# wyf0912/ContextGS

Hardware: AMD Instinct MI355X
Metric: views/sec fwd+bwd @1920×1080, 1M anchors (higher is better)
Workload: dtype f32

## Files before the change

contextgs_amd/_lib.py:

```python
from __future__ import annotations

import ctypes as C
import os
import threading

_HERE = os.path.dirname(os.path.abspath(__file__))
LIB_PATH = os.environ.get("CGS_LIB_PATH") or os.path.join(_HERE, "libcgs_hip.so")

_lib = None
_lock = threading.Lock()

c_void_p, c_int, c_int32, c_int64, c_size_t, c_float = C.c_void_p, C.c_int, C.c_int32, C.c_int64, C.c_size_t, C.c_float


class RasterCfg(C.Structure):
    _fields_ = [
        ("image_height", c_int32),
        ("image_width", c_int32),
        ("tanfovx", c_float),
        ("tanfovy", c_float),
        ("scale_modifier", c_float),
        ("prefiltered", c_int32),
        ("debug", c_int32),
        ("viewmatrix", c_void_p),
# ... 16 lines not shown
        ("step_size", c_float),
        ("bias2_sqrt", c_float),
        ("eps", c_float),
        ("weight_decay", c_float),
    ]


class RateSubLevel(C.Structure):
    _fields_ = [("in_dim", c_int32), ("use_clamp", c_int32), ("n", c_int64), ("m", c_int64)] + [
        (k, c_void_p) for k in ("X", "loc", "W1", "b1", "W2", "b2", "yf", "ys", "yo", "Q", "masks", "x_means", "sums3", "g_sums3",
                                "side_f", "side_s", "side_o", "side_Q", "dx_sub", "d_masks", "dW1", "db1", "dW2", "db2")]


_BWD_HEAD = [C.POINTER(RasterCfg), c_int64, c_int64]
_BWD_WS = [c_void_p, c_size_t, c_void_p, c_size_t, c_void_p, c_size_t]
_BWD_TAIL = [c_void_p, c_size_t, c_void_p]
_BWD_FORMS = _BWD_HEAD + [c_void_p] * 3 + [c_int32] * 2 + [c_void_p] * 5 + _BWD_WS + [c_void_p]
_BWD_MAPS = _BWD_FORMS + [c_void_p] * 3
_BWD_OUT = [c_void_p] * 8 + _BWD_TAIL
_BWD_FEAT = [c_void_p, c_int32, c_void_p, c_void_p]

SIGNATURES = {
    "cgs_version": (c_int, []),
    "cgs_last_error": (C.c_char_p, []),
    "cgs_filter": (c_int, [C.POINTER(RasterCfg), c_int64, c_void_p, c_void_p, c_void_p, c_void_p, c_void_p]),
    "cgs_filter_voxel": (c_int, [C.POINTER(RasterCfg), c_int64, c_void_p, c_void_p, c_int64, c_int, c_void_p, c_void_p, c_void_p]),
    "cgs_raster_geom_bytes": (c_size_t, [c_int64]),
    "cgs_raster_bin_bytes": (c_size_t, [c_int64, c_int64]),
    "cgs_raster_img_bytes": (c_size_t, [c_int32, c_int32]),
    "cgs_raster_bwd_scratch_bytes": (c_size_t, [c_int64]),
    "cgs_raster_preprocess": (c_int, [C.POINTER(RasterCfg), c_int64, c_void_p, c_void_p, c_void_p, c_void_p,
                                      c_void_p, c_void_p, c_size_t, c_void_p, C.POINTER(c_int64), c_void_p]),
    "cgs_raster_preprocess_launch": (c_int, [C.POINTER(RasterCfg), c_int64, c_void_p, c_void_p, c_void_p, c_void_p,
                                             c_void_p, c_void_p, c_size_t, c_void_p, c_void_p, C.POINTER(C.c_uint64)]),
    "cgs_raster_preprocess_launch_ex": (c_int, [C.POINTER(RasterCfg), c_int64, c_void_p, c_void_p, c_void_p, c_int32, c_int32,
                                                c_void_p, c_void_p, c_void_p, c_void_p, c_void_p, c_size_t, c_void_p, c_void_p,
                                                C.POINTER(C.c_uint64)]),
    "cgs_raster_backward_ex": (c_int, _BWD_FORMS + _BWD_OUT),
    "cgs_raster_render_aux": (c_int, [C.POINTER(RasterCfg), c_int64, c_int64, c_void_p, c_size_t, c_void_p, c_size_t,
                                      c_void_p, c_size_t, c_void_p, c_void_p, c_void_p, c_void_p]),
    "cgs_raster_backward_aux": (c_int, _BWD_MAPS + _BWD_OUT),
    "cgs_raster_bwd_aux_scratch_bytes": (c_size_t, [c_int64]),
    "cgs_raster_preprocess_launch_opt": (c_int, [C.POINTER(RasterCfg), c_int64, c_void_p, c_void_p, c_void_p, c_int32, c_int32,
                                                 c_void_p, c_void_p, c_void_p, c_void_p, c_void_p, c_size_t, c_void_p, c_void_p,
                                                 C.POINTER(C.c_uint64), C.c_uint32]),
    "cgs_raster_backward_opt": (c_int, _BWD_MAPS + _BWD_OUT + [C.c_uint32]),
    "cgs_raster_render_features": (c_int, [C.POINTER(RasterCfg), c_int64, c_int64, c_void_p, c_size_t, c_void_p, c_size_t,
                                           c_void_p, c_size_t, c_void_p, c_int32, c_void_p, c_void_p]),
    "cgs_raster_backward_feat": (c_int, _BWD_MAPS + _BWD_OUT + [C.c_uint32] + _BWD_FEAT),
    "cgs_raster_bwd_abs_scratch_bytes": (c_size_t, [c_int64]),
    "cgs_raster_backward_abs": (c_int, _BWD_MAPS + _BWD_OUT + [C.c_uint32] + _BWD_FEAT),
    "cgs_raster_bwd_det_bytes": (c_size_t, [c_int64, c_int64, c_int32]),
    "cgs_raster_backward_det": (c_int, _BWD_MAPS + _BWD_OUT + [C.c_uint32, c_int32, c_void_p, c_size_t]),
    "cgs_raster_render_geom": (c_int, [C.POINTER(RasterCfg), c_int64, c_int64, c_void_p, c_size_t, c_void_p, c_size_t,
                                       c_void_p, c_size_t, c_void_p, c_void_p, c_void_p, c_void_p, c_void_p]),
    "cgs_raster_backward_geom": (c_int, _BWD_MAPS + _BWD_OUT + [C.c_uint32] + _BWD_FEAT + [c_void_p] * 4),
    "cgs_raster_contrib": (c_int, [C.POINTER(RasterCfg), c_int64, c_int64, c_void_p, c_size_t, c_void_p, c_size_t, c_void_p,
                                   c_size_t, c_void_p, c_int64] + [c_void_p] * 8),
    "cgs_raster_camera_bytes": (c_size_t, [c_int64]),
    "cgs_raster_camera_backward": (c_int, [C.POINTER(RasterCfg), c_int64, c_void_p, c_void_p, c_int32, c_int32, c_void_p, c_void_p,
                                           c_void_p, c_void_p, c_void_p, c_void_p, c_size_t, c_void_p, c_void_p, C.c_uint32,
                                           c_void_p, c_void_p, c_void_p, c_void_p, c_size_t, c_void_p]),
    "cgs_gaussian_normals_fwd": (c_int, [C.POINTER(RasterCfg), c_int64] + [c_void_p] * 5),
    "cgs_gaussian_normals_bwd": (c_int, [C.POINTER(RasterCfg), c_int64] + [c_void_p] * 6),
    "cgs_depth_normals_fwd": (c_int, [c_int32, c_int32, c_float, c_float, c_float] + [c_void_p] * 3),
    "cgs_depth_normals_bwd": (c_int, [c_int32, c_int32, c_float, c_float, c_float] + [c_void_p] * 4),
    "cgs_normal_consistency_fwd": (c_int, [c_int32, c_int32, c_float, c_float, c_float] + [c_void_p] * 5),
    "cgs_normal_consistency_bwd": (c_int, [c_int32, c_int32, c_float, c_float, c_float] + [c_void_p] * 7),
    "cgs_filter_cov": (c_int,[C.POINTER(RasterCfg), c_int64, c_void_p, c_void_p, c_void_p, c_void_p]),
    "cgs_raster_preprocess_wait": (c_int, [C.c_uint64, C.POINTER(c_int64)]),
    "cgs_raster_preprocess_wait2": (c_int, [C.c_uint64, C.POINTER(c_int64), C.POINTER(c_int)]),
    "cgs_debug_set_depth_keys_full": (c_int, [c_int]),
    "cgs_sort_depth_keys": (c_int, [c_void_p, c_void_p, c_void_p, c_void_p, c_void_p, c_int64, c_void_p, c_size_t, c_void_p,
                                    C.c_uint32, c_void_p]),
    "cgs_raster_render_spec": (c_int, [C.POINTER(RasterCfg), c_int64, c_int64, c_void_p, c_size_t, c_void_p, c_size_t,
                                       c_void_p, c_size_t, c_void_p, c_void_p]),
    "cgs_raster_render": (c_int, [C.POINTER(RasterCfg), c_int64, c_int64, c_void_p, c_size_t, c_void_p, c_size_t,
                                  c_void_p, c_size_t, c_void_p, c_void_p]),
    "cgs_raster_backward": (c_int, _BWD_HEAD + [c_void_p] * 6 + _BWD_WS + [c_void_p] * 7 + _BWD_TAIL),
    "cgs_raster_preprocess_expand_launch": (c_int, [C.POINTER(RasterCfg), c_int64, c_int] + [c_void_p] * 9 + [c_int64, c_void_p,
                                                    c_void_p, c_void_p, c_void_p, c_size_t, c_void_p, c_void_p, C.POINTER(C.c_uint64)]),
    "cgs_raster_stats": (c_int, [C.POINTER(RasterCfg), c_void_p, c_size_t, c_void_p, c_void_p]),
    "cgs_debug_set_bin_mode": (c_int, [c_int]),
    "cgs_debug_bin_compare": (c_int, [C.POINTER(RasterCfg), c_int64, c_int64, c_int64, c_void_p, c_size_t, c_void_p, c_size_t,
                                      c_void_p, c_size_t, c_void_p, c_size_t, c_void_p, c_void_p, c_void_p]),
    "cgs_build_info": (C.c_char_p, []),
    "cgs_scan_scratch_bytes": (c_size_t, [c_int64]),
    "cgs_scan_exclusive_u32": (c_int, [c_void_p, c_void_p, c_int64, c_void_p, c_size_t, c_void_p]),
    "cgs_sort_scratch_bytes": (c_size_t, [c_int64]),
    "cgs_sort_pairs_u32": (c_int, [c_void_p, c_void_p, c_void_p, c_void_p, c_void_p, c_void_p, c_int64, c_int, c_int,
                                   c_void_p, c_size_t, c_void_p]),
    "cgs_quantize_anchor": (c_int, [c_void_p, c_void_p, c_void_p, c_int64, c_int, c_void_p, c_void_p, c_void_p]),
    "cgs_ste_multistep": (c_int, [c_void_p, c_void_p, c_int64, c_int64, c_int, c_void_p, c_void_p]),
    "cgs_entropy_gaussian_fwd": (c_int, [c_void_p, c_void_p, c_void_p, c_void_p, c_int64, c_int64, c_void_p, c_int,
                                         c_void_p, c_void_p]),
    "cgs_entropy_gaussian_bwd": (c_int, [c_void_p, c_void_p, c_void_p, c_void_p, c_int64, c_int64, c_void_p, c_int,
                                         c_void_p, c_void_p, c_void_p, c_void_p, c_void_p, c_void_p]),
    "cgs_mlp2_forward": (c_int, [c_int, c_int, c_int, c_int, c_void_p, c_int64, c_void_p, c_void_p, c_void_p, c_void_p,
                                 c_void_p, c_int64, c_void_p, c_int64, c_void_p]),
    "cgs_mlp2_backward": (c_int, [c_int, c_int, c_int, c_int, c_void_p, c_int64, c_void_p, c_void_p, c_void_p, c_void_p, c_void_p,
                                  c_int64, c_void_p, c_void_p, c_int64, c_int, c_void_p, c_void_p, c_void_p, c_void_p,
                                  c_void_p, c_void_p, c_int64, c_void_p, c_size_t, c_void_p]),
    "cgs_mlp2_backward_rows": (c_int, [c_int, c_int, c_int, c_int, c_void_p, c_int64, c_void_p, c_void_p, c_void_p, c_void_p,
                                       c_void_p, c_int64, c_void_p, c_void_p, c_int64, c_int, c_void_p, c_void_p, c_void_p,
                                       c_void_p, c_void_p, c_void_p, c_void_p, c_int64, c_void_p, c_size_t, c_void_p]),
    "cgs_mlp_wgrad_scratch_bytes": (c_size_t, []),
    "cgs_mlp2_wgrad": (c_int, [c_int, c_int, c_int, c_void_p, c_int64, c_void_p, c_void_p, c_int64, c_void_p, c_void_p, c_void_p,
                               c_void_p, c_void_p, c_int64, c_void_p, c_size_t, c_void_p]),
    "cgs_anchor_mlp3_wgrad": (c_int, [c_void_p, c_int64] + [c_void_p] * 9 + [c_int64, c_void_p, c_size_t, c_void_p]),
    "cgs_anchor_mlp3_forward": (c_int, [c_void_p, c_int64, c_void_p, c_void_p, c_void_p, c_void_p, c_void_p, c_void_p,
                                        c_void_p, c_void_p, c_int64, c_void_p]),
    "cgs_anchor_mlp3_backward": (c_int, [c_void_p, c_int64, c_void_p, c_void_p, c_void_p, c_void_p, c_void_p, c_void_p,
                                         c_void_p, c_void_p, c_void_p, c_int64, c_void_p, c_void_p, c_void_p, c_void_p,
                                         c_void_p, c_void_p, c_void_p, c_int64, c_void_p, c_size_t, c_void_p]),
    "cgs_anchor_mlp3_forward_rows": (c_int, [c_void_p] * 13 + [c_int64, c_void_p]),
    "cgs_anchor_mlp3_backward_rows": (c_int, [c_void_p] * 22 + [c_int64, c_void_p, c_size_t, c_void_p]),
    "cgs_anchor_mlp3_forward_rows_t": (c_int, [c_void_p] * 13 + [c_int64, c_int, c_void_p]),
    "cgs_anchor_mlp3_backward_rows_t": (c_int, [c_void_p] * 22 + [c_int64, c_int, c_void_p, c_size_t, c_void_p]),
    "cgs_rowcat_fwd": (c_int, [c_int, c_void_p, c_void_p, c_void_p, c_void_p, c_int64, c_void_p, c_void_p]),
    "cgs_rowcat_bwd": (c_int, [c_int, c_void_p, c_void_p, c_void_p, c_void_p, c_void_p, c_int64, c_void_p, c_void_p]),
    "cgs_anchor_mlp3_layout": (c_int, [c_void_p]),
    "cgs_gather_rows_segmented": (c_int, [c_int, c_void_p, c_void_p, c_void_p, c_void_p, c_int64, c_int, c_void_p, c_void_p]),
    "cgs_scatter_rows_sorted": (c_int, [c_void_p, c_void_p, c_int64, c_int64, c_int, c_void_p, c_void_p]),
    "cgs_add_rows": (c_int, [c_void_p, c_void_p, c_int64, c_int64, c_int, c_void_p, c_void_p]),
    "cgs_weighted_sum_scratch_bytes": (c_size_t, []),
    "cgs_weighted_sum_fwd": (c_int, [c_void_p, c_void_p, c_int64, c_void_p, c_float, c_void_p, c_size_t, c_void_p, c_void_p]),
    "cgs_weighted_sum_bwd": (c_int, [c_void_p, c_void_p, c_int64, c_float, c_void_p, c_void_p, c_void_p]),
    "cgs_gather_rows": (c_int, [c_void_p, c_void_p, c_int64, c_int, c_void_p, c_void_p]),
    "cgs_mark_rows": (c_int, [c_void_p, c_int64, c_int64, C.c_uint32, c_void_p, c_void_p]),
    "cgs_zero_unmarked_rows": (c_int, [c_void_p, C.c_uint32, c_int64, c_int, c_void_p, c_void_p, c_void_p]),
    "cgs_rowcat_fwd_masked": (c_int, [c_int, c_void_p, c_void_p, c_void_p, c_void_p, c_void_p, c_int64, c_void_p, c_void_p]),
    "cgs_rowcat_bwd_masked": (c_int, [c_int, c_void_p, c_void_p, c_void_p, c_void_p, c_void_p, c_void_p, c_int64, c_void_p,
                                      c_void_p]),
    "cgs_ctx_gather_bwd": (c_int, [c_void_p, c_int64, c_int64, c_void_p, c_void_p, c_void_p, c_void_p, c_void_p, c_void_p,
                                   c_int, c_int, c_int, c_void_p]),
    "cgs_ctx_gather_bwd_acc": (c_int, [c_void_p, c_int64, c_int64, c_void_p, c_void_p, c_void_p, c_void_p, c_void_p, c_void_p,
                                       c_int, c_int, c_int, c_int, c_void_p]),
    "cgs_noise_quant_fwd": (c_int, [c_void_p, c_void_p, c_void_p, c_void_p, c_void_p, c_int64, c_int, c_int, c_int,
                                    C.c_uint64, c_float, c_float, c_float, c_void_p, c_void_p, c_void_p, c_void_p,
                                    c_void_p, c_void_p]),
    "cgs_hyper_noise_gather": (c_int, [c_void_p, c_void_p, c_int64, c_int, C.c_uint64, c_void_p, c_void_p]),
    "cgs_eb_bits_scratch_bytes": (c_size_t, []),
    "cgs_eb_bits_fwd": (c_int, [c_void_p, c_void_p, c_void_p, c_int64, c_int, c_void_p, c_size_t, c_void_p, c_void_p]),
    "cgs_eb_bits_bwd": (c_int, [c_void_p, c_void_p, c_void_p, c_void_p, c_int64, c_int, c_void_p, c_void_p, c_void_p]),
    "cgs_rate_finish_fwd": (c_int, [c_void_p, c_int, c_void_p, c_float, C.c_double, C.c_double, C.c_double, c_float, c_void_p,
                                    c_void_p, c_void_p]),
    "cgs_rate_finish_bwd": (c_int, [c_void_p, c_int, c_float, C.c_double, C.c_double, C.c_double, c_void_p, c_void_p, c_void_p]),
    "cgs_rate_finish_bwd4": (c_int, [c_void_p, c_void_p, c_void_p, c_void_p, c_int, c_float, C.c_double, C.c_double, C.c_double, c_void_p,
                                     c_void_p, c_void_p]),
    "cgs_ctx_choose_blocks": (c_size_t, [c_int64]),
    "cgs_ctx_choose_flags": (c_int, [c_void_p, c_int64, c_void_p, c_void_p, C.c_uint64, c_float, c_void_p, c_void_p, c_void_p,
                                     c_void_p, c_int, c_void_p, c_void_p, c_void_p, c_void_p]),
    "cgs_ctx_choose_slot_ints": (c_int, []),
    "cgs_ctx_choose_flags_slots": (c_int, [c_void_p, c_int64, c_void_p, c_void_p, C.c_uint64, c_float, c_void_p, c_void_p, c_void_p,
                                           c_void_p, c_int, c_void_p, c_void_p, c_void_p, c_int, c_void_p]),
    "cgs_ctx_choose_compact": (c_int, [c_void_p, c_void_p, c_void_p, c_int64, c_void_p, c_int, c_void_p, c_void_p, c_void_p,
                                       c_void_p, c_void_p, c_void_p]),
    "cgs_means_accum_doubles": (c_size_t, []),
    "cgs_means_finalize": (c_int, [c_void_p, c_int64, c_int64, c_int64, c_void_p, c_void_p]),
    "cgs_noise_quant_bwd": (c_int, [c_void_p, c_void_p, c_void_p, c_void_p, c_void_p, c_int64, c_int, c_int, c_int,
                                    C.c_uint64, c_float, c_float, c_float, c_void_p, c_void_p, c_void_p, c_void_p,
                                    c_void_p, c_void_p, c_void_p, c_void_p, c_void_p, c_void_p, c_void_p]),
    "cgs_ctx_level_fwd": (c_int, [c_int, c_void_p, c_int64, c_void_p, c_void_p, c_void_p, c_void_p, c_int64, c_void_p, c_void_p,
                                  c_int64] + [c_void_p] * 8 + [C.c_uint64, c_float, c_float, c_float] + [c_void_p] * 7),
    "cgs_ctx_level_bwd_scratch_bytes": (c_size_t, []),
    "cgs_ctx_level_bwd": (c_int, [c_int] + [c_void_p] * 9 + [c_int64, C.c_uint64, c_float, c_float, c_float, c_void_p, c_int64] +
# ... 183 lines not shown
```

contextgs_amd/csrc/tile_bin.hip:

```cpp
#include "cgs_internal.h"
#include "buf_access.h"

#define TB_THREADS 256
#define TB_ITEMS 16
#define TB_TILE (TB_THREADS * TB_ITEMS)
#define TB_WAVES (TB_THREADS / CGS_WAVE)
#define TB_MAXR 256
#ifndef TB_XCD_MAP
#define TB_XCD_MAP 0
#endif

int cgs_scan_exclusive_u32_total(const uint32_t *in, uint32_t *out, int64_t n, void *scratch, size_t scratch_bytes,
                                 uint32_t *grand_total, hipStream_t stream);

namespace {

#ifndef GR_ITEMS
#define GR_ITEMS 2
#endif
__global__ void __launch_bounds__(256)
    gather_rects_kernel(int64_t P, const uint32_t *__restrict__ order, const uint2 *__restrict__ rect,
                        uint32_t *__restrict__ rect_lo, uint32_t *__restrict__ rect_hi, uint32_t *__restrict__ cnt) {
    const int64_t blk = cgs_xcd_item((P + 256 * GR_ITEMS - 1) / (256 * GR_ITEMS));
    if (blk < 0) return;
// ... 9 lines not shown
        const int64_t i = i0 + 256 * k;
        if (i < P) {
            rect_lo[i] = rc[k].x;
            rect_hi[i] = rc[k].y;
            const uint32_t w = (rc[k].y & 0xFFFFu) - (rc[k].x & 0xFFFFu), h = (rc[k].y >> 16) - (rc[k].x >> 16);
            cnt[i] = w * h;
        }
    }
}

__global__ void __launch_bounds__(256)
    block_first_kernel(int64_t nb, int64_t P, const uint32_t *__restrict__ offsets, uint32_t *__restrict__ bf, int nt,
                       uint2 *__restrict__ ranges, const uint32_t *__restrict__ R_dev, uint32_t R_cap) {
    const int64_t b = (int64_t)blockIdx.x * 256 + threadIdx.x;
    if (b < nt) ranges[b] = make_uint2(0u, 0u);
    if (R_dev) nb = ((int64_t)min(*R_dev, R_cap) + TB_TILE - 1) / TB_TILE;
    if (b > nb) return;
    if (b == nb) { bf[b] = (uint32_t)(P - 1); return; }
    const uint32_t target = (uint32_t)(b * TB_TILE);
    int64_t lo = 0, hi = P;
    while (lo < hi) {
        const int64_t mid = (lo + hi) >> 1;
        if (offsets[mid] <= target) lo = mid + 1; else hi = mid;
    }
    bf[b] = (uint32_t)(lo - 1);
}

__device__ __forceinline__ void build_owner_index(uint32_t *sidx, uint32_t *swave , uint32_t base, uint32_t i_lo,
                                                  uint32_t i_hi, int64_t P, uint32_t R,
                                                  const uint32_t *__restrict__ offsets) {
    const int tid = threadIdx.x, lane = tid & 63, wave = tid >> 6;
#pragma unroll
    for (int k = 0; k < TB_ITEMS; ++k) sidx[k * TB_THREADS + tid] = 0u;
    __syncthreads();
    for (uint32_t i = i_lo + 1u + (uint32_t)tid; i <= i_hi; i += TB_THREADS) {
        const uint32_t o = offsets[i];
        const uint32_t on = (int64_t)i + 1 < P ? offsets[i + 1] : R;
        if (on > o && o > base && o - base < (uint32_t)TB_TILE) sidx[o - base] = i - i_lo;
    }
    __syncthreads();
    uint32_t v[TB_ITEMS];
    uint32_t run = 0;
#pragma unroll
    for (int k = 0; k < TB_ITEMS; ++k) {
        v[k] = sidx[tid * TB_ITEMS + k];
        run = max(run, v[k]);
    }
    uint32_t inc = run;
#pragma unroll
    for (int d = 1; d < 64; d <<= 1) {
        const uint32_t o = (uint32_t)__shfl_up((int)inc, d, 64);
        if (lane >= d) inc = max(inc, o);
    }
    if (lane == 63) swave[wave] = inc;
    __syncthreads();
    uint32_t pre = (uint32_t)__shfl_up((int)inc, 1, 64);
    if (lane == 0) pre = 0;
#pragma unroll
    for (int w = 0; w < TB_WAVES; ++w) pre = (w < wave) ? max(pre, swave[w]) : pre;
    run = pre;
#pragma unroll
    for (int k = 0; k < TB_ITEMS; ++k) {
        run = max(run, v[k]);
        sidx[tid * TB_ITEMS + k] = run;
    }
    __syncthreads();
}

struct TbPair { uint32_t key, i, mask; };

#define BK_W 8
#define BK_H 4
#define BK_TILES (BK_W * BK_H)

__device__ __forceinline__ void bucket_rect(uint32_t lo, uint32_t hi, uint32_t &cx0, uint32_t &cy0, uint32_t &cw, uint32_t &ch) {
    const uint32_t x0 = lo & 0xFFFFu, y0 = lo >> 16, x1 = hi & 0xFFFFu, y1 = hi >> 16;
    const bool some = x1 > x0 && y1 > y0;
    cx0 = x0 / BK_W;
    cy0 = y0 / BK_H;
    cw = some ? (x1 + BK_W - 1) / BK_W - cx0 : 0u;
    ch = some ? (y1 + BK_H - 1) / BK_H - cy0 : 0u;
}

template <bool COARSE>
__device__ __forceinline__ TbPair gen_pair(uint32_t j, uint32_t base, uint32_t i_lo, const uint32_t *sidx,
                                           const uint32_t *__restrict__ offsets, const uint32_t *__restrict__ rect_lo,
                                           const uint32_t *__restrict__ rect_hi, uint32_t tiles_x) {
    TbPair p;
    p.i = i_lo + sidx[j - base];
    p.mask = 0u;
    const uint32_t local = j - offsets[p.i];
    const uint32_t lo = rect_lo[p.i], hi = rect_hi[p.i];
    uint32_t x0 = lo & 0xFFFFu, y0 = lo >> 16, w = (hi & 0xFFFFu) - x0, h = 0;
    if (COARSE) bucket_rect(lo, hi, x0, y0, w, h);
    uint32_t q = (uint32_t)((float)local * __builtin_amdgcn_rcpf((float)w));
    int32_t r = (int32_t)(local - q * w);
    if (r < 0) { --q; r += (int32_t)w; }
    if (r >= (int32_t)w) { ++q; r -= (int32_t)w; }
    p.key = (y0 + q) * tiles_x + x0 + (uint32_t)r;
    if (COARSE) {
        const int32_t tx0 = (int32_t)((x0 + (uint32_t)r) * BK_W), ty0 = (int32_t)((y0 + q) * BK_H);
        const int32_t c0 = max((int32_t)(lo & 0xFFFFu) - tx0, 0), c1 = min((int32_t)(hi & 0xFFFFu) - tx0, BK_W);
        const int32_t r0 = max((int32_t)(lo >> 16) - ty0, 0), r1 = min((int32_t)(hi >> 16) - ty0, BK_H);
        const uint32_t cols = ((1u << c1) - 1u) & ~((1u << c0) - 1u), rows = ((1u << r1) - 1u) & ~((1u << r0) - 1u);
        p.mask = cols * ((rows & 1u) | ((rows & 2u) << 7) | ((rows & 4u) << 14) | ((rows & 8u) << 21));
    }
    return p;
}

template <bool GEN, bool COARSE = false>
__global__ void __launch_bounds__(TB_THREADS)
    tb_hist_kernel(const uint16_t *__restrict__ keys, const uint32_t *__restrict__ offsets,
                   const uint32_t *__restrict__ rect_lo, const uint32_t *__restrict__ rect_hi,
                   const uint32_t *__restrict__ bf, int64_t P, uint32_t R, uint32_t tiles_x,
                   uint32_t *__restrict__ hist , int shift, int nbits, const uint32_t *__restrict__ R_dev,
                   uint32_t ncol, int xcd) {
    const int64_t col_ = xcd ? cgs_xcd_item((int64_t)ncol) : (int64_t)blockIdx.x;
    if (col_ < 0) return;
    const uint32_t col = (uint32_t)col_;
    if (R_dev) R = min(*R_dev, R);
    __shared__ uint32_t h[TB_MAXR];
    __shared__ uint32_t sidx[GEN ? TB_TILE : 1];
    __shared__ uint32_t swave[TB_WAVES];
    const int tid = threadIdx.x;
    const uint32_t mask = (1u << nbits) - 1u;
    h[tid] = 0;
    const uint32_t nblk = (R + (uint32_t)TB_TILE - 1u) / (uint32_t)TB_TILE, per = max(1u, (nblk + ncol - 1u) / ncol);
    const uint32_t b0 = col * per, b1 = min(nblk, b0 + per);
    __syncthreads();
    for (uint32_t blk = b0; blk < b1; ++blk) {
        const uint32_t base = blk * (uint32_t)TB_TILE;
        uint32_t i_lo = 0;
        if (GEN) {
            i_lo = bf[blk];
            build_owner_index(sidx, swave, base, i_lo, bf[blk + 1], P, R, offsets);
        }
#pragma unroll 4
        for (int k = 0; k < TB_ITEMS; ++k) {
            const uint32_t j = base + (uint32_t)(k * TB_THREADS + tid);
            if (j < R) {
                const uint32_t key = GEN ? gen_pair<COARSE>(j, base, i_lo, sidx, offsets, rect_lo, rect_hi, tiles_x).key
                                         : (uint32_t)keys[j];
                atomicAdd(&h[(key >> shift) & mask], 1u);
            }
        }
        __syncthreads();
    }
    if (tid < (1 << nbits)) hist[(int64_t)tid * ncol + col] = h[tid];
}

template <bool GEN, bool FINAL, int NBITS, bool COARSE = false>
__global__ void __launch_bounds__(TB_THREADS)
    tb_scatter_kernel(const uint16_t *__restrict__ keys_in, const uint32_t *__restrict__ vals_in,
                      const uint32_t *__restrict__ offsets, const uint32_t *__restrict__ rect_lo,
                      const uint32_t *__restrict__ rect_hi, const uint32_t *__restrict__ order,
                      const uint32_t *__restrict__ bf, int64_t P, uint32_t R, uint32_t tiles_x,
                      uint16_t *__restrict__ keys_out, uint32_t *__restrict__ vals_out, uint2 *__restrict__ ranges,
                      const uint32_t *__restrict__ hist_scanned, int shift, const uint32_t *__restrict__ R_dev,
                      uint32_t ncol, int xcd, const uint32_t *__restrict__ digit_totals, uint32_t *__restrict__ mask_out = nullptr) {
    const int64_t col_ = xcd ? cgs_xcd_item((int64_t)ncol) : (int64_t)blockIdx.x;
    if (col_ < 0) return;
    const uint32_t col = (uint32_t)col_;
    if (R_dev) R = min(*R_dev, R);
    constexpr int nbits = NBITS;
    const uint32_t nblk = (R + (uint32_t)TB_TILE - 1u) / (uint32_t)TB_TILE, per = max(1u, (nblk + ncol - 1u) / ncol);
    const uint32_t b0 = col * per, b1 = min(nblk, b0 + per);
    if (b0 >= b1) return;
    __shared__ uint32_t wcnt[TB_WAVES][TB_MAXR];
    __shared__ uint32_t lstart[TB_MAXR], gbase[TB_MAXR];
    __shared__ uint32_t wsum[TB_WAVES];
    __shared__ uint32_t stage[TB_TILE + TB_TILE / 2];
    uint32_t *sval = stage;
    uint16_t *skey = (uint16_t *)(stage + TB_TILE);
    const int tid = threadIdx.x, lane = tid & 63, wave = tid >> 6;
    const uint32_t mask = (1u << nbits) - 1u;
    uint32_t gcur = tid < (1 << nbits) ? hist_scanned[(int64_t)tid * ncol + col] : 0u;
    if (digit_totals) {
        const uint32_t gt = tid < (1 << nbits) ? digit_totals[tid] : 0u;
        uint32_t ginc = gt;
#pragma unroll
        for (int o = 1; o < 64; o <<= 1) {
            const uint32_t up = __shfl_up(ginc, o, 64);
            if (lane >= o) ginc += up;
        }
        if (lane == 63) wsum[wave] = ginc;
        __syncthreads();
        uint32_t goff = 0;
#pragma unroll
        for (int w = 0; w < TB_WAVES; ++w) goff += (w < wave) ? wsum[w] : 0u;
        gcur += goff + ginc - gt;
    }
    for (uint32_t blk = b0; blk < b1; ++blk) {
    __syncthreads();
#pragma unroll
    for (int w = 0; w < TB_WAVES; ++w) wcnt[w][tid] = 0;
    const uint32_t base = blk * (uint32_t)TB_TILE;
    uint32_t i_lo = 0;
    if (GEN) {
        i_lo = bf[blk];
        build_owner_index(stage, wsum, base, i_lo, bf[blk + 1], P, R, offsets);
    } else {
        __syncthreads();
    }
    const uint32_t wbase = base + (uint32_t)wave * (TB_TILE / TB_WAVES);
    uint32_t key[TB_ITEMS], val[TB_ITEMS], rank[TB_ITEMS], tmask[COARSE ? TB_ITEMS : 1];
    volatile uint32_t *my = wcnt[wave];
    const uint64_t lt_mask = (1ull << lane) - 1ull;
#pragma unroll
    for (int r = 0; r < TB_ITEMS; ++r) {
        const uint32_t j = wbase + (uint32_t)(r * 64 + lane);
        const bool valid = j < R;
        key[r] = 0xFFFFu;
        val[r] = 0u;
        if (valid) {
            if (GEN) {
                const TbPair p = gen_pair<COARSE>(j, base, i_lo, stage, offsets, rect_lo, rect_hi, tiles_x);
                key[r] = p.key;
                val[r] = order[p.i];
                if (COARSE) tmask[r] = p.mask;
            } else {
                key[r] = keys_in[j];
                val[r] = vals_in[j];
            }
        }
        const uint32_t d = (key[r] >> shift) & mask;
        uint64_t peers = __ballot(valid);
#pragma unroll
        for (int b = 0; b < nbits; ++b) {
            const bool bit = (d >> b) & 1u;
            const uint64_t m = __ballot(bit);
            peers &= bit ? m : ~m;
        }
        uint32_t old = 0;
        rank[r] = 0;
        if (valid) {
            const int leader = __builtin_ctzll(peers);
            if (lane == leader) {
                old = my[d];
                my[d] = old + (uint32_t)__builtin_popcountll(peers);
            }
            old = __shfl(old, leader, 64);
            rank[r] = old + (uint32_t)__builtin_popcountll(peers & lt_mask);
        }
    }
    __syncthreads();
    {
        const int d = tid;
        uint32_t tot = 0;
#pragma unroll
        for (int w = 0; w < TB_WAVES; ++w) tot += wcnt[w][d];
        uint32_t inc = tot;
#pragma unroll
        for (int o = 1; o < 64; o <<= 1) {
            const uint32_t up = __shfl_up(inc, o, 64);
            if (lane >= o) inc += up;
        }
        if (lane == 63) wsum[wave] = inc;
        __syncthreads();
        uint32_t woff = 0;
#pragma unroll
        for (int w = 0; w < TB_WAVES; ++w) woff += (w < wave) ? wsum[w] : 0u;
        uint32_t run = woff + inc - tot;
        lstart[d] = run;
        gbase[d] = gcur - run;
        gcur += tot;
#pragma unroll
        for (int w = 0; w < TB_WAVES; ++w) {
            const uint32_t c = wcnt[w][d];
            wcnt[w][d] = run;
            run += c;
        }
    }
    __syncthreads();
#pragma unroll
    for (int r = 0; r < TB_ITEMS; ++r) {
        const uint32_t j = wbase + (uint32_t)(r * 64 + lane);
        if (j < R) {
            const uint32_t d = (key[r] >> shift) & mask;
            const uint32_t slot = wcnt[wave][d] + rank[r];
            skey[slot] = (uint16_t)key[r];
            sval[slot] = val[r];
            if (COARSE) mask_out[gbase[d] + slot] = tmask[r];
        }
    }
    __syncthreads();
    const int count = (int)min((uint32_t)TB_TILE, R - base);
    for (int j = tid; j < count; j += TB_THREADS) {
        const uint32_t k = skey[j];
        const uint32_t d = (k >> shift) & mask;
        const uint32_t pos = gbase[d] + (uint32_t)j;
        vals_out[pos] = sval[j];
        if (FINAL && !COARSE) {
            if (j + 1 == count || (uint32_t)skey[j + 1] != k) atomicMax(&ranges[k].y, pos + 1u);
        } else if (!FINAL) {
            keys_out[pos] = (uint16_t)k;
        }
    }
    }
// ... 155 lines not shown
        uint32_t acc[BK_TILES];
#pragma unroll
        for (int j = 0; j < BK_TILES; ++j) acc[j] = 0;
        const ClBuf bm = cl_buf(masks + q.s, (uint64_t)(q.e - q.s) * 4u);
        const uint32_t n = q.e - q.s;
        uint32_t m_next = (uint32_t)__builtin_amdgcn_raw_buffer_load_b32(bm, lane * 4, 0, 0);
        for (uint32_t p0 = 0; p0 < n; p0 += CGS_WAVE) {
            const uint32_t m = m_next;
            m_next = (uint32_t)__builtin_amdgcn_raw_buffer_load_b32(bm, (int)((p0 + CGS_WAVE + (uint32_t)lane) * 4u), 0, 0);
#pragma unroll
            for (int j = 0; j < BK_TILES; ++j) acc[j] += (uint32_t)__builtin_popcountll(__ballot(m & (1u << j)));
        }
        uint32_t mine = 0;
#pragma unroll
        for (int j = 0; j < BK_TILES; ++j) mine = lane == j ? acc[j] : mine;
        if (lane < BK_TILES) {
            const int t = bk_tile(q.b, lane, bx, tiles_x, tiles_y);
            if (t >= 0) counts[tab[BK_TAB_TS + t] + q.k] = mine;
        }
    }
}

__global__ void __launch_bounds__(BK_THREADS)
    bk_fill_kernel(const uint32_t *__restrict__ ids, const uint32_t *__restrict__ masks, const uint32_t *__restrict__ tab,
                   uint32_t tiles_x, uint32_t tiles_y, uint32_t bx, const uint32_t *__restrict__ counts,
                   const uint32_t *__restrict__ S, uint32_t cap, uint32_t *__restrict__ out, uint2 *__restrict__ ranges) {
    __shared__ uint32_t cs[BK_MAXB + 1];
    const int tid = threadIdx.x, lane = tid & 63, wave = tid >> 6;
    for (int i = tid; i <= BK_MAXB; i += BK_THREADS) cs[i] = tab[BK_TAB_CS + i];
    const uint32_t nch = tab[BK_TAB_NCH];
    const ClBuf bout = cl_buf(out, (uint64_t)cap * 4u);
    __syncthreads();
    for (uint32_t c = blockIdx.x * BK_WAVES + (uint32_t)wave; c < nch; c += gridDim.x * BK_WAVES) {
        const BkChunk q = bk_chunk(c, cs, tab);
        uint32_t first = 0;
        if (lane < BK_TILES) {
            const int t = bk_tile(q.b, lane, bx, tiles_x, tiles_y);
            if (t >= 0) {
                const uint32_t slot = tab[BK_TAB_TS + t];
                first = S[slot + q.k];
                if (q.k == 0) {
                    const uint32_t last = slot + (cs[q.b + 1] - cs[q.b]) - 1u;
                    const uint32_t end = min(S[last] + counts[last], cap);
                    if (end > first) ranges[t] = make_uint2(first, end);
                }
            }
        }
        uint32_t gb[BK_TILES];
#pragma unroll
        for (int j = 0; j < BK_TILES; ++j) gb[j] = (uint32_t)__builtin_amdgcn_readlane((int)first, j) * 4u;
        const ClBuf bm = cl_buf(masks + q.s, (uint64_t)(q.e - q.s) * 4u), bi = cl_buf(ids + q.s, (uint64_t)(q.e - q.s) * 4u);
        const uint32_t n = q.e - q.s;
        uint32_t m_next = (uint32_t)__builtin_amdgcn_raw_buffer_load_b32(bm, lane * 4, 0, 0);
        uint32_t id_next = (uint32_t)__builtin_amdgcn_raw_buffer_load_b32(bi, lane * 4, 0, 0);
        asm volatile("" : "+v"(m_next), "+v"(id_next));
        for (uint32_t p0 = 0; p0 < n; p0 += CGS_WAVE) {
            const uint32_t m = m_next, id = id_next;
            const int on = (int)((p0 + CGS_WAVE + (uint32_t)lane) * 4u);
            m_next = (uint32_t)__builtin_amdgcn_raw_buffer_load_b32(bm, on, 0, 0);
            id_next = (uint32_t)__builtin_amdgcn_raw_buffer_load_b32(bi, on, 0, 0);
#pragma unroll
            for (int j = 0; j < BK_TILES; ++j) {
                const bool bit = m & (1u << j);
                const uint64_t bal = __ballot(bit);
                const uint32_t rank = __builtin_amdgcn_mbcnt_hi((uint32_t)(bal >> 32), __builtin_amdgcn_mbcnt_lo((uint32_t)bal, 0u));
                __builtin_amdgcn_raw_buffer_store_b32((int)id, bout, (int)cl_sel(bit, gb[j] + rank * 4u), 0, 0);
                gb[j] += (uint32_t)__builtin_popcountll(bal) * 4u;
            }
        }
    }
}

}

int cgs_launch_gather_rects(int64_t P, CgsGeom &g, hipStream_t stream) {
    if (P == 0) return CGS_OK;
    hipLaunchKernelGGL(gather_rects_kernel, dim3(cgs_xcd_grid((P + 256 * GR_ITEMS - 1) / (256 * GR_ITEMS))), dim3(256), 0, stream, P,
                       (const uint32_t *)g.order, (const uint2 *)g.rect, g.sort_b, g.sort_d, g.sort_a);
    CGS_CHECK_HIP(hipGetLastError());
    return CGS_OK;
}

bool cgs_tile_bin16_ok(int tile_bits) { return tile_bits <= 16; }

int cgs_launch_tile_bin16(const cgs_raster_cfg *cfg, int64_t P, int64_t R, int tile_bits, CgsGeom &g, CgsBin &b, CgsImg &im,
                          hipStream_t stream, const uint32_t *R_dev) {
    const int nt = cgs_tiles_x(cfg) * cgs_tiles_y(cfg);
    if (R == 0 || P == 0) {
        CGS_CHECK_HIP(hipMemsetAsync(im.ranges, 0, (size_t)nt * sizeof(uint2), stream));
        return CGS_OK;
    }
    if (R >= (1ll << 32) - TB_TILE) { cgs_set_error("tile binning: pair count out of range"); return CGS_ERR_ARG; }
    const int64_t nb = (R + TB_TILE - 1) / TB_TILE;
    const int bits_b = tile_bits > 8 ? tile_bits / 2 : 0;
    const int bits_a = tile_bits - bits_b;
    uint32_t *bf = b.tile_key_b;
    uint16_t *key_a = (uint16_t *)b.tile_key_a;
    uint32_t *hist = (uint32_t *)b.scratch;
    const size_t hist_bytes = cgs_align_up((size_t)TB_MAXR * nb * sizeof(uint32_t), 256);
    if (b.scratch_bytes < hist_bytes + cgs_scan_scratch_bytes((int64_t)TB_MAXR * nb)) {
        cgs_set_error("tile binning: scratch too small");
        return CGS_ERR_WORKSPACE;
    }
    char *scan_scratch = (char *)b.scratch + hist_bytes;
    const size_t scan_bytes = b.scratch_bytes - hist_bytes;
    const uint32_t tiles_x = (uint32_t)cgs_tiles_x(cfg);
    const uint32_t *offsets = g.offsets, *rlo = g.sort_b, *rhi = g.sort_d, *order = g.order;
    int rc;
    uint32_t *totals = (uint32_t *)scan_scratch;
    (void)scan_bytes;
    const unsigned grid = TB_XCD_MAP ? cgs_xcd_grid(nb) : (unsigned)nb;
#define TB_SCATTER_N(GEN, FINAL, N, KIN, VIN, KOUT, VOUT, SHIFT)                                                          \
    hipLaunchKernelGGL((tb_scatter_kernel<GEN, FINAL, N>), dim3(grid), dim3(TB_THREADS), 0, stream, KIN, VIN,             \
                       offsets, rlo, rhi, order, (const uint32_t *)bf, P, (uint32_t)R, tiles_x, KOUT, VOUT, im.ranges,    \
                       (const uint32_t *)hist, SHIFT, R_dev, (uint32_t)nb, TB_XCD_MAP, (const uint32_t *)totals)
#define TB_SCATTER(GEN, FINAL, NB, KIN, VIN, KOUT, VOUT, SHIFT)                                                           \
    do { switch (NB) {                                                                                                    \
        case 1: TB_SCATTER_N(GEN, FINAL, 1, KIN, VIN, KOUT, VOUT, SHIFT); break;                                          \
        case 2: TB_SCATTER_N(GEN, FINAL, 2, KIN, VIN, KOUT, VOUT, SHIFT); break;                                          \
        case 3: TB_SCATTER_N(GEN, FINAL, 3, KIN, VIN, KOUT, VOUT, SHIFT); break;                                          \
        case 4: TB_SCATTER_N(GEN, FINAL, 4, KIN, VIN, KOUT, VOUT, SHIFT); break;                                          \
        case 5: TB_SCATTER_N(GEN, FINAL, 5, KIN, VIN, KOUT, VOUT, SHIFT); break;                                          \
        case 6: TB_SCATTER_N(GEN, FINAL, 6, KIN, VIN, KOUT, VOUT, SHIFT); break;                                          \
        case 7: TB_SCATTER_N(GEN, FINAL, 7, KIN, VIN, KOUT, VOUT, SHIFT); break;                                          \
        default: TB_SCATTER_N(GEN, FINAL, 8, KIN, VIN, KOUT, VOUT, SHIFT); break;                                         \
    } } while (0)
    {
        CgsProfScope prof(CGS_PROF_EMIT_PAIRS, stream);
        const int64_t nthr = nb + 1 > nt ? nb + 1 : nt;
        hipLaunchKernelGGL(block_first_kernel, dim3((unsigned)((nthr + 255) / 256)), dim3(256), 0, stream, nb, P, offsets, bf,
                           nt, im.ranges, R_dev, (uint32_t)R);
        hipLaunchKernelGGL(tb_hist_kernel<true>, dim3(grid), dim3(TB_THREADS), 0, stream,
                           (const uint16_t *)nullptr, offsets, rlo, rhi, (const uint32_t *)bf, P, (uint32_t)R, tiles_x,
                           hist, 0, bits_a, R_dev, (uint32_t)nb, TB_XCD_MAP);
        CGS_CHECK_HIP(hipGetLastError());
        if ((rc = cgs_launch_digit_scan(hist, totals, 1 << bits_a, nb, stream))) return rc;
        if (bits_b)
            TB_SCATTER(true, false, bits_a, (const uint16_t *)nullptr, (const uint32_t *)nullptr, key_a, b.gid_a, 0);
        else
            TB_SCATTER(true, true, bits_a, (const uint16_t *)nullptr, (const uint32_t *)nullptr, (uint16_t *)nullptr,
                       b.gid_sorted, 0);
        CGS_CHECK_LAUNCH(stream, cfg->debug);
    }
    if (bits_b) {
        CgsProfScope prof(CGS_PROF_TILE_SORT, stream);
        hipLaunchKernelGGL(tb_hist_kernel<false>, dim3(grid), dim3(TB_THREADS), 0, stream,
                           (const uint16_t *)key_a, offsets, rlo, rhi, (const uint32_t *)bf, P, (uint32_t)R, tiles_x, hist,
                           bits_a, bits_b, R_dev, (uint32_t)nb, TB_XCD_MAP);
        CGS_CHECK_HIP(hipGetLastError());
        if ((rc = cgs_launch_digit_scan(hist, totals, 1 << bits_b, nb, stream))) return rc;
        TB_SCATTER(false, true, bits_b, (const uint16_t *)key_a, (const uint32_t *)b.gid_a, (uint16_t *)nullptr,
                   b.gid_sorted, bits_a);
        CGS_CHECK_LAUNCH(stream, cfg->debug);
    }
    {
        CgsProfScope prof(CGS_PROF_RANGES, stream);
        hipLaunchKernelGGL(ranges_fix_kernel, dim3(1), dim3(1024), 0, stream, nt, im.ranges);
        CGS_CHECK_LAUNCH(stream, cfg->debug);
    }
    return CGS_OK;
}

static void bk_dims(const cgs_raster_cfg *cfg, uint32_t &bx, uint32_t &by) {
    bx = (uint32_t)(cgs_tiles_x(cfg) + BK_W - 1) / BK_W;
    by = (uint32_t)(cgs_tiles_y(cfg) + BK_H - 1) / BK_H;
}
// ... 105 lines not shown
```

include/cgs.h:

```cpp
#ifndef CGS_H
#define CGS_H

#include <stddef.h>
#include <stdint.h>

#ifdef __cplusplus
extern "C" {
#endif

#define CGS_VERSION 100

#define CGS_OK 0
#define CGS_ERR_ARG 1
#define CGS_ERR_HIP 2
#define CGS_ERR_WORKSPACE 3
#define CGS_ERR_BOUNDS 4
#define CGS_ERR_RESPEC 5

int cgs_version(void);
const char *cgs_last_error(void);


typedef struct cgs_raster_cfg {
    int32_t image_height;
// ... 197 lines not shown

int cgs_raster_render_geom(const cgs_raster_cfg *cfg, int64_t P, int64_t num_rendered,
                           void *geom_ws, size_t geom_bytes, void *bin_ws, size_t bin_bytes,
                           void *img_ws, size_t img_bytes, float *out_distortion,
                           float *out_median_depth, int32_t *out_median_id,
                           float *out_moments, void *stream);
int cgs_raster_backward_geom(const cgs_raster_cfg *cfg, int64_t P,
                             int64_t num_rendered, const float *means3D,
                             const float *colors, const float *shs,
                             int32_t sh_degree, int32_t sh_coeffs,
                             const float *opacities, const float *scales,
                             const float *rotations, const float *cov3D,
                             const int32_t *radii, void *geom_ws, size_t geom_bytes,
                             void *bin_ws, size_t bin_bytes, void *img_ws,
                             size_t img_bytes, const float *dL_dout,
                             const float *dL_ddepth, const float *dL_dinvdepth,
                             const float *dL_dalpha, float *dL_dmeans3D,
                             float *dL_dmeans2D, float *dL_dcolors,
                             float *dL_dopacities, float *dL_dshs,
                             float *dL_dscales, float *dL_drotations,
                             float *dL_dcov3D, void *scratch,
                             size_t scratch_bytes, void *stream, uint32_t opts,
                             const float *features, int32_t C,
                             const float *dL_dfeatures_map, float *dL_dfeatures,
                             const float *moments, const int32_t *median_id,
                             const float *dL_ddistortion, const float *dL_dmedian_depth);

int cgs_raster_contrib(const cgs_raster_cfg *cfg, int64_t P, int64_t num_rendered,
                       void *geom_ws, size_t geom_bytes, void *bin_ws, size_t bin_bytes, void *img_ws, size_t img_bytes,
                       const int32_t *slot, int64_t n_slots,
                       float *acc_weight, float *acc_max_weight, int64_t *acc_pixels, int64_t *acc_top_pixels,
                       int32_t *out_top_id, float *out_top_weight, int32_t *out_count, void *stream);

#define CGS_RASTER_CAMERA_MAPS 2u
size_t cgs_raster_camera_bytes(int64_t P);
int cgs_raster_camera_backward(const cgs_raster_cfg *cfg, int64_t P,
                               const float *means3D, const float *shs,
                               int32_t sh_degree, int32_t sh_coeffs,
                               const float *opacities, const float *scales,
                               const float *rotations, const float *cov3D,
                               const int32_t *radii, const void *scratch,
                               size_t scratch_bytes, const float *dL_dcolors,
                               const float *dL_dopacities, uint32_t opts,
                               float *dL_dviewmatrix, float *dL_dprojmatrix,
                               float *dL_dcampos, void *work, size_t work_bytes,
                               void *stream);

int cgs_gaussian_normals_fwd(const cgs_raster_cfg *cfg, int64_t P, const float *means3D,
                             const float *scales, const float *rotations,
                             float *out_normals, void *stream);
int cgs_gaussian_normals_bwd(const cgs_raster_cfg *cfg, int64_t P, const float *means3D,
                             const float *scales, const float *rotations,
                             const float *dL_dnormals, float *dL_drotations, void *stream);
int cgs_depth_normals_fwd(int32_t H, int32_t W, float tanfovx, float tanfovy, float eps,
                          const float *depth, float *out_normals, void *stream);
int cgs_depth_normals_bwd(int32_t H, int32_t W, float tanfovx, float tanfovy, float eps,
                          const float *depth, const float *dL_dnormals, float *dL_ddepth,
                          void *stream);
int cgs_normal_consistency_fwd(int32_t H, int32_t W, float tanfovx, float tanfovy, float eps,
                               const float *normals, const float *depth, const float *weight,
                               float *out_error, void *stream);
int cgs_normal_consistency_bwd(int32_t H, int32_t W, float tanfovx, float tanfovy, float eps,
                               const float *normals, const float *depth, const float *weight,
                               const float *dL_derror, float *dL_dnormals, float *dL_ddepth,
                               void *stream);

int cgs_raster_preprocess_expand_launch(const cgs_raster_cfg *cfg, int64_t n_anchor, int K,
                                        const uint8_t *flags, const uint32_t *pos, const float *anchor,
                                        const float *gscaling, const float *offsets,
                                        const float *neural_opacity, const float *color_in,
                                        const float *cov_in, const int64_t *src_row, int64_t P,
                                        float *scaling_out, float *xyz_out, float *rot_out, void *geom_ws,
                                        size_t geom_bytes, int32_t *radii, void *stream, uint64_t *ticket);
size_t cgs_raster_bwd_scratch_bytes(int64_t P);

int cgs_raster_stats(const cgs_raster_cfg *cfg, void *img_ws, size_t img_bytes,
                     int64_t *stats_out, void *stream);
int cgs_debug_bin_compare(const cgs_raster_cfg *cfg, int64_t P, int64_t R,
                          int64_t R_ws, void *geom_ws, size_t geom_bytes,
                          void *bin_ws, size_t bin_bytes, void *img_ws,
                          size_t img_bytes, void *bin_ws2, size_t bin_bytes2,
                          void *ranges2, int64_t *out2, void *stream);
int cgs_debug_set_bin_mode(int mode);
const char *cgs_build_info(void);


size_t cgs_scan_scratch_bytes(int64_t n);
int cgs_scan_exclusive_u32(const uint32_t *in, uint32_t *out, int64_t n,
                           void *scratch, size_t scratch_bytes, void *stream);

size_t cgs_sort_scratch_bytes(int64_t n);
int cgs_sort_pairs_u32(const uint32_t *keys_in, const uint32_t *vals_in,
                       uint32_t *keys_out, uint32_t *vals_out,
                       uint32_t *keys_tmp, uint32_t *vals_tmp, int64_t n,
                       int bit_lo, int bit_hi, void *scratch,
                       size_t scratch_bytes, void *stream);
int cgs_sort_depth_keys(const uint32_t *keys_in, uint32_t *keys_out, uint32_t *vals_out,
                        uint32_t *keys_tmp, uint32_t *vals_tmp, int64_t n, void *scratch,
                        size_t scratch_bytes, uint32_t *overflow, uint32_t epoch, void *stream);

int cgs_prof_enable(int on);
int cgs_prof_count(void);
const char *cgs_prof_name(int id);
int cgs_prof_read(int id, double *total_ms, int64_t *launches);


int cgs_quantize_anchor(const float *anchors, const float *min_v,
                        const float *max_v, int64_t N, int round_digits,
                        float *anchors_q, float *quantized, void *stream);

int cgs_ste_multistep(const float *x, const float *Q, int64_t n, int64_t q_div,
                      int use_clamp, float *out, void *stream);

int cgs_entropy_gaussian_fwd(const float *x, const float *mean,
                             const float *scale, const float *Q, int64_t n,
                             int64_t q_div, const float *x_mean, int use_clamp,
                             float *bits, void *stream);
int cgs_entropy_gaussian_bwd(const float *x, const float *mean,
                             const float *scale, const float *Q, int64_t n,
                             int64_t q_div, const float *x_mean, int use_clamp,
                             const float *g_bits, float *g_x, float *g_mean,
                             float *g_scale, float *g_Q, void *stream);

int cgs_mlp2_forward(int in, int hid, int out, int act, const float *X,
                     int64_t ldx, const float *W1, const float *b1,
                     const float *W2, const float *b2, float *Y, int64_t ldy,
                     float *H, int64_t n, void *stream);
size_t cgs_mlp_wgrad_scratch_bytes(void);
int cgs_mlp2_backward(int in, int hid, int out, int act, const float *X,
                      int64_t ldx, const float *W1, const float *b1, const float *W2,
                      const float *Y, const float *dY, int64_t ldy,
                      const float *H, float *dX, int64_t lddx,
                      int accumulate_dx, float *dZ1, float *dZ2, float *dW1,
                      float *db1, float *dW2, float *db2, int64_t n,
                      void *scratch, size_t scratch_bytes, void *stream);
int cgs_mlp2_backward_rows(int in, int hid, int out, int act, const float *X, int64_t ldx,
                           const float *W1, const float *b1, const float *W2, const float *Y,
                           const float *dY, int64_t ldy, const float *H, float *dX, int64_t lddx,
                           int accumulate_dx, const int64_t *dx_rows, float *dZ1, float *dZ2,
                           float *dW1, float *db1, float *dW2, float *db2, int64_t n,
                           void *scratch, size_t scratch_bytes, void *stream);
int cgs_mlp2_wgrad(int in, int hid, int out, const float *X, int64_t ldx, const float *H,
                   const float *dZ2, int64_t lddz2, const float *dZ1, float *dW1, float *db1,
                   float *dW2, float *db2, int64_t n, void *scratch, size_t scratch_bytes,
                   void *stream);

int cgs_rowcat_fwd(int nsrc, const void *const *data, const int64_t *const *idx,
                   const int *width, const int *ld, int64_t n, float *out,
                   void *stream);
int cgs_rowcat_bwd(int nsrc, void *const *ddata, const int64_t *const *idx,
                   const int *width, const int *ld, const int *mode, int64_t n,
                   const float *dout, void *stream);
int cgs_rowcat_fwd_masked(int nsrc, const void *const *data, const int64_t *const *idx,
                          const uint8_t *const *rowmask, const int *width, const int *ld,
                          int64_t n, float *out, void *stream);
int cgs_rowcat_bwd_masked(int nsrc, void *const *ddata, const int64_t *const *idx,
                          const uint8_t *const *rowmask, const int *width, const int *ld,
                          const int *mode, int64_t n, const float *dout, void *stream);

int cgs_scatter_rows_sorted(const float *g, const int64_t *idx, int64_t n, int64_t N, int w,
                            float *out, void *stream);
int cgs_add_rows(const float *g, const int64_t *idx, int64_t n, int64_t N, int w, float *out,
                 void *stream);
int cgs_gather_rows(const float *x, const int64_t *idx, int64_t n, int w,
                    float *out, void *stream);
int cgs_mark_rows(const int64_t *idx, int64_t n, int64_t n_full, uint32_t gen,
// ... 449 lines not shown
```

Before: 175.0.

## Expand tile pairs per owner with long-owner wave/block redistribution in tile binning

```diff
diff --git a/contextgs_amd/_lib.py b/contextgs_amd/_lib.py
--- a/contextgs_amd/_lib.py
+++ b/contextgs_amd/_lib.py
@@ -122,6 +122,7 @@
                                                     c_void_p, c_void_p, c_void_p, c_size_t, c_void_p, c_void_p, C.POINTER(C.c_uint64)]),
     "cgs_raster_stats": (c_int, [C.POINTER(RasterCfg), c_void_p, c_size_t, c_void_p, c_void_p]),
     "cgs_debug_set_bin_mode": (c_int, [c_int]),
+    "cgs_debug_tile_bin_long_owner": (c_int, []),
     "cgs_debug_bin_compare": (c_int, [C.POINTER(RasterCfg), c_int64, c_int64, c_int64, c_void_p, c_size_t, c_void_p, c_size_t,
                                       c_void_p, c_size_t, c_void_p, c_size_t, c_void_p, c_void_p, c_void_p]),
     "cgs_build_info": (C.c_char_p, []),
diff --git a/contextgs_amd/csrc/tile_bin.hip b/contextgs_amd/csrc/tile_bin.hip
--- a/contextgs_amd/csrc/tile_bin.hip
+++ b/contextgs_amd/csrc/tile_bin.hip
@@ -115,6 +115,14 @@
     ch = some ? (y1 + BK_H - 1) / BK_H - cy0 : 0u;
 }
 
+__device__ __forceinline__ void tb_divmod(uint32_t local, uint32_t w, uint32_t &q, uint32_t &r) {
+    q = (uint32_t)((float)local * __builtin_amdgcn_rcpf((float)w));
+    int32_t rr = (int32_t)(local - q * w);
+    if (rr < 0) { --q; rr += (int32_t)w; }
+    if (rr >= (int32_t)w) { ++q; rr -= (int32_t)w; }
+    r = (uint32_t)rr;
+}
+
 template <bool COARSE>
 __device__ __forceinline__ TbPair gen_pair(uint32_t j, uint32_t base, uint32_t i_lo, const uint32_t *sidx,
                                            const uint32_t *__restrict__ offsets, const uint32_t *__restrict__ rect_lo,
@@ -126,13 +134,11 @@
     const uint32_t lo = rect_lo[p.i], hi = rect_hi[p.i];
     uint32_t x0 = lo & 0xFFFFu, y0 = lo >> 16, w = (hi & 0xFFFFu) - x0, h = 0;
     if (COARSE) bucket_rect(lo, hi, x0, y0, w, h);
-    uint32_t q = (uint32_t)((float)local * __builtin_amdgcn_rcpf((float)w));
-    int32_t r = (int32_t)(local - q * w);
-    if (r < 0) { --q; r += (int32_t)w; }
-    if (r >= (int32_t)w) { ++q; r -= (int32_t)w; }
-    p.key = (y0 + q) * tiles_x + x0 + (uint32_t)r;
+    uint32_t q, r;
+    tb_divmod(local, w, q, r);
+    p.key = (y0 + q) * tiles_x + x0 + r;
     if (COARSE) {
-        const int32_t tx0 = (int32_t)((x0 + (uint32_t)r) * BK_W), ty0 = (int32_t)((y0 + q) * BK_H);
+        const int32_t tx0 = (int32_t)((x0 + r) * BK_W), ty0 = (int32_t)((y0 + q) * BK_H);
         const int32_t c0 = max((int32_t)(lo & 0xFFFFu) - tx0, 0), c1 = min((int32_t)(hi & 0xFFFFu) - tx0, BK_W);
         const int32_t r0 = max((int32_t)(lo >> 16) - ty0, 0), r1 = min((int32_t)(hi >> 16) - ty0, BK_H);
         const uint32_t cols = ((1u << c1) - 1u) & ~((1u << c0) - 1u), rows = ((1u << r1) - 1u) & ~((1u << r0) - 1u);
@@ -141,6 +147,110 @@
     return p;
 }
 
+#ifndef TB_LONG_OWNER
+#define TB_LONG_OWNER 20
+#endif
+#define TB_OWNERS 4
+#define TB_LONG_MAX (TB_THREADS)
+#define TB_HUGE_OWNER (TB_TILE / TB_WAVES)
+static_assert(TB_TILE / (TB_LONG_OWNER + 1) <= TB_LONG_MAX, "the long-owner list holds every long owner of a block");
+struct TbLongList { uint32_t n, i[TB_LONG_MAX], se[TB_LONG_MAX]; };
+
+template <bool WITH_ID, class Emit>
+__device__ __forceinline__ void expand_block(TbLongList &ll, uint32_t base, uint32_t end, uint32_t i_lo, uint32_t i_hi, int64_t P,
+                                             uint32_t R, const uint32_t *__restrict__ offsets, const uint32_t *__restrict__ rect_lo,
+                                             const uint32_t *__restrict__ rect_hi, const uint32_t *__restrict__ order,
+                                             uint32_t tiles_x, Emit emit) {
+    const uint32_t tid = threadIdx.x, lane = tid & 63u, wave = tid >> 6;
+    const uint32_t last = (uint32_t)(P - 1);
+    if (tid == 0) ll.n = 0u;
+    __syncthreads();
+    for (uint32_t c = i_lo; c <= i_hi; c += TB_THREADS * TB_OWNERS) {
+        uint32_t o[TB_OWNERS], on[TB_OWNERS], lo[TB_OWNERS], hi[TB_OWNERS], id[TB_OWNERS];
+#pragma unroll
+        for (int k = 0; k < TB_OWNERS; ++k) {
+            const uint32_t ic = min(c + (uint32_t)(k * TB_THREADS) + tid, i_hi);
+            o[k] = offsets[ic];
+            on[k] = offsets[min(ic + 1u, last)];
+            lo[k] = rect_lo[ic];
+            hi[k] = rect_hi[ic];
+            id[k] = WITH_ID ? order[ic] : 0u;
+        }
+#pragma unroll
+        for (int k = 0; k < TB_OWNERS; ++k) {
+            const uint32_t i = c + (uint32_t)(k * TB_THREADS) + tid;
+            const uint32_t s = max(o[k], base), e = min(i >= last ? R : on[k], end);
+            const uint32_t n = (i <= i_hi && e > s) ? e - s : 0u;
+            if (n > (uint32_t)TB_LONG_OWNER) {
+                const uint32_t at = atomicAdd(&ll.n, 1u);
+                if (at < (uint32_t)TB_LONG_MAX) {
+                    ll.i[at] = i;
+                    ll.se[at] = (s - base) | ((e - base) << 16);
+                }
+            } else if (n) {
+                const uint32_t x0 = lo[k] & 0xFFFFu, y0 = lo[k] >> 16, w = (hi[k] & 0xFFFFu) - x0;
+                uint32_t q, x;
+                tb_divmod(s - o[k], w, q, x);
+                uint32_t key = (y0 + q) * tiles_x + x0 + x, slot = s - base;
+                for (uint32_t t = 0; t < n; ++t) {
+                    emit(slot + t, key, id[k]);
+                    ++x;
+                    ++key;
+                    if (x == w) { x = 0u; key += tiles_x - w; }
+                }
+            }
+        }
+    }
+    __syncthreads();
+    const uint32_t nl = min(ll.n, (uint32_t)TB_LONG_MAX);
+    for (uint32_t e0 = 0; e0 < nl; e0 += CGS_WAVE * TB_WAVES) {
+        const uint32_t en = e0 + lane * TB_WAVES + wave;
+        const bool have = en < nl;
+        const uint32_t i = have ? ll.i[en] : i_lo, se = have ? ll.se[en] : 0u;
+        const uint32_t o = offsets[i], lo = rect_lo[i], hi = rect_hi[i], id = WITH_ID ? order[i] : 0u;
+        const uint32_t s = se & 0xFFFFu, e = se >> 16;
+        uint64_t m = __ballot(have && e - s <= (uint32_t)TB_HUGE_OWNER);
+        while (m) {
+            const int src = __builtin_ctzll(m);
+            m &= m - 1ull;
+            const uint32_t so = (uint32_t)__builtin_amdgcn_readlane((int)o, src);
+            const uint32_t ss = (uint32_t)__builtin_amdgcn_readlane((int)s, src);
+            const uint32_t sn = (uint32_t)__builtin_amdgcn_readlane((int)e, src);
+            const uint32_t slo = (uint32_t)__builtin_amdgcn_readlane((int)lo, src);
+            const uint32_t shi = (uint32_t)__builtin_amdgcn_readlane((int)hi, src);
+            const uint32_t sid = (uint32_t)__builtin_amdgcn_readlane((int)id, src);
+            const uint32_t sx0 = slo & 0xFFFFu, sw = (shi & 0xFFFFu) - sx0, skey0 = (slo >> 16) * tiles_x + sx0;
+            const uint32_t first = base - so;
+            for (uint32_t j = ss + lane; j < sn; j += CGS_WAVE) {
+                uint32_t q, r;
+                tb_divmod(first + j, sw, q, r);
+                emit(j, skey0 + q * tiles_x + r, sid);
+            }
+        }
+    }
+    for (uint32_t e0 = 0; e0 < nl; e0 += CGS_WAVE) {
+        const uint32_t en = e0 + lane;
+        const uint32_t se = en < nl ? ll.se[en] : 0u;
+        uint64_t m = __ballot((se >> 16) - (se & 0xFFFFu) > (uint32_t)TB_HUGE_OWNER);
+        while (m) {
+            const uint32_t src = e0 + (uint32_t)__builtin_ctzll(m);
+            m &= m - 1ull;
+            const uint32_t i = ll.i[src], sse = ll.se[src];
+            const uint32_t so = offsets[i], slo = rect_lo[i], shi = rect_hi[i], sid = WITH_ID ? order[i] : 0u;
+            const uint32_t sx0 = slo & 0xFFFFu, sw = (shi & 0xFFFFu) - sx0, skey0 = (slo >> 16) * tiles_x + sx0;
+            const uint32_t first = base - so;
+            for (uint32_t j = (sse & 0xFFFFu) + tid; j < (sse >> 16); j += TB_THREADS) {
+                uint32_t q, r;
+                tb_divmod(first + j, sw, q, r);
+                emit(j, skey0 + q * tiles_x + r, sid);
+            }
+        }
+    }
+}
+
+#ifndef TB_HCOPIES
+#define TB_HCOPIES 4
+#endif
 template <bool GEN, bool COARSE = false>
 __global__ void __launch_bounds__(TB_THREADS)
     tb_hist_kernel(const uint16_t *__restrict__ keys, const uint32_t *__restrict__ offsets,
@@ -152,17 +262,28 @@
     if (col_ < 0) return;
     const uint32_t col = (uint32_t)col_;
     if (R_dev) R = min(*R_dev, R);
-    __shared__ uint32_t h[TB_MAXR];
-    __shared__ uint32_t sidx[GEN ? TB_TILE : 1];
+    constexpr int HC = GEN ? 1 : TB_HCOPIES;
+    __shared__ uint32_t h[TB_MAXR * HC];
+    __shared__ uint32_t sidx[GEN && COARSE ? TB_TILE : 1];
     __shared__ uint32_t swave[TB_WAVES];
     const int tid = threadIdx.x;
     const uint32_t mask = (1u << nbits) - 1u;
-    h[tid] = 0;
+#pragma unroll
+    for (int c = 0; c < HC; ++c) h[c * TB_THREADS + tid] = 0;
+    const uint32_t hc = (uint32_t)tid & (uint32_t)(HC - 1);
     const uint32_t nblk = (R + (uint32_t)TB_TILE - 1u) / (uint32_t)TB_TILE, per = max(1u, (nblk + ncol - 1u) / ncol);
     const uint32_t b0 = col * per, b1 = min(nblk, b0 + per);
     __syncthreads();
     for (uint32_t blk = b0; blk < b1; ++blk) {
         const uint32_t base = blk * (uint32_t)TB_TILE;
+        if constexpr (GEN && !COARSE) {
+            __shared__ TbLongList llist;
+            expand_block<false>(llist, base, min(base + (uint32_t)TB_TILE, R), bf[blk], bf[blk + 1], P, R, offsets, rect_lo, rect_hi,
+                                nullptr, tiles_x,
+                                [&](uint32_t, uint32_t key, uint32_t) { atomicAdd(&h[((key >> shift) & mask) * HC + hc], 1u); });
+            __syncthreads();
+            continue;
+        }
         uint32_t i_lo = 0;
         if (GEN) {
             i_lo = bf[blk];
@@ -174,12 +295,17 @@
             if (j < R) {
                 const uint32_t key = GEN ? gen_pair<COARSE>(j, base, i_lo, sidx, offsets, rect_lo, rect_hi, tiles_x).key
                                          : (uint32_t)keys[j];
-                atomicAdd(&h[(key >> shift) & mask], 1u);
+                atomicAdd(&h[((key >> shift) & mask) * HC + hc], 1u);
             }
         }
         __syncthreads();
     }
-    if (tid < (1 << nbits)) hist[(int64_t)tid * ncol + col] = h[tid];
+    if (tid < (1 << nbits)) {
+        uint32_t sum = 0;
+#pragma unroll
+        for (int c = 0; c < HC; ++c) sum += h[tid * HC + c];
+        hist[(int64_t)tid * ncol + col] = sum;
+    }
 }
 
 template <bool GEN, bool FINAL, int NBITS, bool COARSE = false>
@@ -229,12 +355,15 @@
     for (int w = 0; w < TB_WAVES; ++w) wcnt[w][tid] = 0;
     const uint32_t base = blk * (uint32_t)TB_TILE;
     uint32_t i_lo = 0;
-    if (GEN) {
+    if constexpr (GEN && !COARSE) {
+        __shared__ TbLongList llist;
+        expand_block<true>(llist, base, min(base + (uint32_t)TB_TILE, R), bf[blk], bf[blk + 1], P, R, offsets, rect_lo, rect_hi,
+                           order, tiles_x, [&](uint32_t slot, uint32_t k, uint32_t id) { skey[slot] = (uint16_t)k; sval[slot] = id; });
+    } else if (GEN) {
         i_lo = bf[blk];
         build_owner_index(stage, wsum, base, i_lo, bf[blk + 1], P, R, offsets);
-    } else {
-        __syncthreads();
-    }
+    }
+    if (!GEN || !COARSE) __syncthreads();
     const uint32_t wbase = base + (uint32_t)wave * (TB_TILE / TB_WAVES);
     uint32_t key[TB_ITEMS], val[TB_ITEMS], rank[TB_ITEMS], tmask[COARSE ? TB_ITEMS : 1];
     volatile uint32_t *my = wcnt[wave];
@@ -246,7 +375,10 @@
         key[r] = 0xFFFFu;
         val[r] = 0u;
         if (valid) {
-            if (GEN) {
+            if constexpr (GEN && !COARSE) {
+                key[r] = skey[j - base];
+                val[r] = sval[j - base];
+            } else if (GEN) {
                 const TbPair p = gen_pair<COARSE>(j, base, i_lo, stage, offsets, rect_lo, rect_hi, tiles_x);
                 key[r] = p.key;
                 val[r] = order[p.i];
@@ -568,6 +700,8 @@
 }
 
 bool cgs_tile_bin16_ok(int tile_bits) { return tile_bits <= 16; }
+
+extern "C" int cgs_debug_tile_bin_long_owner(void) { return TB_LONG_OWNER; }
 
 int cgs_launch_tile_bin16(const cgs_raster_cfg *cfg, int64_t P, int64_t R, int tile_bits, CgsGeom &g, CgsBin &b, CgsImg &im,
                           hipStream_t stream, const uint32_t *R_dev) {
diff --git a/include/cgs.h b/include/cgs.h
--- a/include/cgs.h
+++ b/include/cgs.h
@@ -303,6 +303,7 @@
                           size_t img_bytes, void *bin_ws2, size_t bin_bytes2,
                           void *ranges2, int64_t *out2, void *stream);
 int cgs_debug_set_bin_mode(int mode);
+int cgs_debug_tile_bin_long_owner(void);
 const char *cgs_build_info(void);
 
 
```

New measurement: 176.1, median of 6. No clear change (+0.6%).
